# facebookresearch/foundpose

Measured on AMD Instinct MI355X. Metric: detections/sec (ViT+kNN match) on 518^2 crops vs 10k-template bank, higher is better.
Workload: dtype bf16

## Files before the change

### foundpose_amd/csrc/common.hpp

```cpp
#pragma once
#include <hip/hip_runtime.h>
#include <stdint.h>

#include <atomic>

typedef __attribute__((ext_vector_type(8))) __bf16 bf16x8;
typedef __attribute__((ext_vector_type(4))) __bf16 bf16x4;
typedef __attribute__((ext_vector_type(2))) __bf16 bf16x2;
typedef __attribute__((ext_vector_type(16))) float f32x16;
typedef __attribute__((ext_vector_type(4))) float f32x4;
typedef __attribute__((ext_vector_type(2))) float f32x2;

#define FP_DEVICE __device__ __forceinline__

enum : int {
  FP_OK = 0,
  FP_ERR_INVALID = 1,
  FP_ERR_UNSUPPORTED = 2,
  FP_ERR_HIP = 3,
};

void fp_set_error(const char* fmt, ...);

#define FP_REQUIRE(cond, ...)              \
// ... 2 lines not shown
      fp_set_error(__VA_ARGS__);           \
      return FP_ERR_INVALID;               \
    }                                      \
  } while (0)

#define FP_CHECK_LAUNCH(name)                                              \
  do {                                                                     \
    hipError_t e__ = hipGetLastError();                                    \
    if (e__ != hipSuccess) {                                               \
      fp_set_error("%s: launch failed: %s", name, hipGetErrorString(e__)); \
      return FP_ERR_HIP;                                                   \
    }                                                                      \
  } while (0)

FP_DEVICE float bf16_to_f32(__bf16 v) { return (float)v; }

FP_DEVICE float clamp448(float v) { return fminf(fmaxf(v, -448.f), 448.f); }
FP_DEVICE unsigned pack_fp8x4(float v0, float v1, float v2, float v3) {
  int w = __builtin_amdgcn_cvt_pk_fp8_f32(clamp448(v0), clamp448(v1), 0, false);
  return (unsigned)__builtin_amdgcn_cvt_pk_fp8_f32(clamp448(v2), clamp448(v3), w, true);
}
FP_DEVICE float nanmax3(float a, float b, float c) { return __builtin_elementwise_maximum(a, __builtin_elementwise_maximum(b, c)); }
FP_DEVICE unsigned pack_fp8x4(float v0, float v1, float v2, float v3, float& amax) {
  amax = nanmax3(nanmax3(amax, fabsf(v0), fabsf(v1)), fabsf(v2), fabsf(v3));
  return pack_fp8x4(v0, v1, v2, v3);
}
constexpr float FP_F16_MAX = 65504.f, FP_E4M3_MAX = 448.f;
FP_DEVICE void report_saturation(int* sat, int slot, float amax, float limit) {
  if (sat != nullptr && !(amax <= limit)) atomicAdd(sat + slot, 1);
}

FP_DEVICE unsigned pack_bf16x2(float lo, float hi) {
  f32x2 p = {lo, hi};
  return __builtin_bit_cast(unsigned, __builtin_convertvector(p, bf16x2));
}

typedef __attribute__((ext_vector_type(8))) _Float16 f16x8;
typedef __attribute__((ext_vector_type(2))) _Float16 f16x2;
FP_DEVICE unsigned pack_f16x2(float lo, float hi) {
  f32x2 p = {lo, hi};
  return __builtin_bit_cast(unsigned, __builtin_convertvector(p, f16x2));
}
template <bool H16> FP_DEVICE unsigned pack_h2(float lo, float hi) {
  if constexpr (H16) return pack_f16x2(lo, hi);
  else return pack_bf16x2(lo, hi);
}
template <bool H16> FP_DEVICE f32x2 unpack_h2(unsigned w) {
  if constexpr (H16) return __builtin_convertvector(__builtin_bit_cast(f16x2, w), f32x2);
  else return f32x2{__uint_as_float(w << 16), __uint_as_float(w & 0xffff0000u)};
}
template <bool H16> FP_DEVICE f32x16 mfma_h(bf16x8 a, bf16x8 b, f32x16 c) {
  if constexpr (H16) return __builtin_amdgcn_mfma_f32_32x32x16_f16(__builtin_bit_cast(f16x8, a), __builtin_bit_cast(f16x8, b), c, 0, 0, 0);
  else return __builtin_amdgcn_mfma_f32_32x32x16_bf16(a, b, c, 0, 0, 0);
}

FP_DEVICE void split16_pack2(float a, float b, float scale, unsigned& hi, unsigned& lo) {
  a = __builtin_amdgcn_fmed3f(a * scale, -65504.f, 65504.f);
  b = __builtin_amdgcn_fmed3f(b * scale, -65504.f, 65504.f);
  const f16x2 h = __builtin_convertvector(f32x2{a, b}, f16x2);
  const f32x2 hf = __builtin_convertvector(h, f32x2);
  const f16x2 l = __builtin_convertvector(f32x2{a - hf[0], b - hf[1]}, f16x2);
  hi = __builtin_bit_cast(unsigned, h);
  lo = __builtin_bit_cast(unsigned, l);
}
FP_DEVICE void split16_pack2_inrange(float a, float b, float scale, unsigned& hi, unsigned& lo) {
  a *= scale;
  b *= scale;
  const f16x2 h = __builtin_convertvector(f32x2{a, b}, f16x2);
  const f32x2 hf = __builtin_convertvector(h, f32x2);
  const f16x2 l = __builtin_convertvector(f32x2{a - hf[0], b - hf[1]}, f16x2);
  hi = __builtin_bit_cast(unsigned, h);
  lo = __builtin_bit_cast(unsigned, l);
}
FP_DEVICE void split16_pack2(float a, float b, float scale, unsigned& hi, unsigned& lo, float& amax) {
  amax = nanmax3(amax, fabsf(a * scale), fabsf(b * scale));
  split16_pack2(a, b, scale, hi, lo);
}
FP_DEVICE int split16_pos(int c) { return ((c >> 5) << 6) + (c & 31); }

constexpr float FP_SX_HI_SCALE = 0.0078125f, FP_SX_LO_SCALE = 16.f;
constexpr float FP_SX_MAX = 57344.f;
constexpr unsigned FP_SX_MFMA_SCALE = 0x82828282u;
FP_DEVICE int splitx_pos(int c) { return ((c >> 6) << 7) + (c & 63); }
FP_DEVICE int splitx_hi8(int c) { return ((c >> 6) << 8) + 128 + (c & 63); }
FP_DEVICE void splitx_pack2(float a, float b, float scale, unsigned& hi, unsigned& p8) {
  a = __builtin_amdgcn_fmed3f(a * scale, -65504.f, 65504.f);
  b = __builtin_amdgcn_fmed3f(b * scale, -65504.f, 65504.f);
  const f16x2 h = __builtin_convertvector(f32x2{a, b}, f16x2);
  const f32x2 hf = __builtin_convertvector(h, f32x2);
  hi = __builtin_bit_cast(unsigned, h);
  int w = __builtin_amdgcn_cvt_pk_fp8_f32(clamp448(hf[0] * FP_SX_HI_SCALE), clamp448(hf[1] * FP_SX_HI_SCALE), 0, false);
  p8 = (unsigned)__builtin_amdgcn_cvt_pk_fp8_f32(clamp448((a - hf[0]) * FP_SX_LO_SCALE), clamp448((b - hf[1]) * FP_SX_LO_SCALE), w, true);
}
FP_DEVICE void splitx_pack2(float a, float b, float scale, unsigned& hi, unsigned& p8, float& amax) {
  amax = nanmax3(amax, fabsf(a * scale), fabsf(b * scale));
  splitx_pack2(a, b, scale, hi, p8);
}
FP_DEVICE void splitx_store2(char* row, int c, unsigned hi, unsigned p8) {
  *reinterpret_cast<unsigned*>(row + splitx_pos(c) * 2) = hi;
  *reinterpret_cast<unsigned short*>(row + splitx_hi8(c)) = (unsigned short)p8;
  *reinterpret_cast<unsigned short*>(row + splitx_hi8(c) + 64) = (unsigned short)(p8 >> 16);
}
FP_DEVICE void splitx_store4(char* row, int c, unsigned hi01, unsigned p01, unsigned hi23, unsigned p23) {
  *reinterpret_cast<uint2*>(row + splitx_pos(c) * 2) = make_uint2(hi01, hi23);
  *reinterpret_cast<unsigned*>(row + splitx_hi8(c)) = __builtin_amdgcn_perm(p23, p01, 0x05040100u);
  *reinterpret_cast<unsigned*>(row + splitx_hi8(c) + 64) = __builtin_amdgcn_perm(p23, p01, 0x07060302u);
// ... 61 lines not shown
```

### foundpose_amd/csrc/gemm_bf16.hip

```cpp
#include "common.hpp"
#include "kernels.hpp"

namespace {

constexpr int BK = 64;

typedef __attribute__((address_space(3))) void lds_void;

FP_DEVICE int swz(int row) { return (row >> 1) & 7; }

FP_DEVICE unsigned stage_lane_offset(int ld, int lane, int parity) {
  const int row_l = lane >> 3;
  const int chunk = (lane & 7) ^ ((4 * parity + (row_l >> 1)) & 7);
  return (unsigned)(row_l * ld + chunk * 8) * 2u;
}
FP_DEVICE void stage_rows(__amdgpu_buffer_rsrc_t rsrc, unsigned voff, int ld, int row0, int k0, char* lds, int rblk) {
  const unsigned soff = (unsigned)((row0 + rblk * 8) * ld + k0) * 2u;
  __builtin_amdgcn_raw_ptr_buffer_load_lds(rsrc, (lds_void*)(lds + rblk * 1024), 16, voff, soff, 0, 0);
}

FP_DEVICE bf16x8 read_frag(const char* lds, int row, int chunk) {
  return *reinterpret_cast<const bf16x8*>(lds + row * 128 + ((chunk ^ swz(row)) << 4));
}

// ... 32 lines not shown
  const f32x2 phi = __builtin_elementwise_fma(xc, q, f32x2{0.5f, 0.5f});
  return x * phi;
}

FP_DEVICE f32x2 gelu_erf_pk(f32x2 x) {
  const f32x2 hx = x * f32x2{0.5f, 0.5f};
  const f32x2 hax = {__builtin_fabsf(hx[0]), __builtin_fabsf(hx[1])};
  const f32x2 z = hax * f32x2{1.41421356237309504880f, 1.41421356237309504880f};
  const f32x2 den = __builtin_elementwise_fma(z, f32x2{0.3275911f, 0.3275911f}, f32x2{1.f, 1.f});
  const f32x2 t = {__builtin_amdgcn_rcpf(den[0]), __builtin_amdgcn_rcpf(den[1])};
  f32x2 q = f32x2{-0.29844723923966754f, -0.29844723923966754f};
  q = __builtin_elementwise_fma(q, t, f32x2{1.5048025775340452f, 1.5048025775340452f});
  q = __builtin_elementwise_fma(q, t, f32x2{-2.0855161249300567f, -2.0855161249300567f});
  q = __builtin_elementwise_fma(q, t, f32x2{2.040068178110667f, 2.040068178110667f});
  q = __builtin_elementwise_fma(q, t, f32x2{-0.7490454190655901f, -0.7490454190655901f});
  q = __builtin_elementwise_fma(q, t, f32x2{0.4310967998728252f, 0.4310967998728252f});
  q = __builtin_elementwise_fma(q, t, f32x2{0.15704123123125485f, 0.15704123123125485f});
  q = q * t;
  const f32x2 a = z * (z * f32x2{-1.44269504088896340736f, -1.44269504088896340736f});
  const f32x2 e = {__builtin_amdgcn_exp2f(a[0]), __builtin_amdgcn_exp2f(a[1])};
  const f32x2 erfz = __builtin_elementwise_fma(-q, e, f32x2{1.f, 1.f});
  return __builtin_elementwise_fma(hax, erfz, hx);
}

FP_DEVICE float row32_sum(float v) {
  v += __builtin_bit_cast(float, __builtin_amdgcn_update_dpp(0, __builtin_bit_cast(int, v), 0xB1, 0xF, 0xF, true));
  v += __builtin_bit_cast(float, __builtin_amdgcn_update_dpp(0, __builtin_bit_cast(int, v), 0x4E, 0xF, 0xF, true));
  v += __builtin_bit_cast(float, __builtin_amdgcn_update_dpp(0, __builtin_bit_cast(int, v), 0x124, 0xF, 0xF, true));
  v += __builtin_bit_cast(float, __builtin_amdgcn_update_dpp(0, __builtin_bit_cast(int, v), 0x128, 0xF, 0xF, true));
  v += __builtin_bit_cast(float, __builtin_amdgcn_update_dpp(0, __builtin_bit_cast(int, v), 0x142, 0xA, 0xF, true));
  return v;
}

FP_DEVICE float row16_sum(float v) {
  v += __builtin_bit_cast(float, __builtin_amdgcn_update_dpp(0, __builtin_bit_cast(int, v), 0xB1, 0xF, 0xF, true));
  v += __builtin_bit_cast(float, __builtin_amdgcn_update_dpp(0, __builtin_bit_cast(int, v), 0x4E, 0xF, 0xF, true));
  v += __builtin_bit_cast(float, __builtin_amdgcn_update_dpp(0, __builtin_bit_cast(int, v), 0x124, 0xF, 0xF, true));
  v += __builtin_bit_cast(float, __builtin_amdgcn_update_dpp(0, __builtin_bit_cast(int, v), 0x128, 0xF, 0xF, true));
  return v;
}

typedef __attribute__((ext_vector_type(8))) int i32x8;
typedef __attribute__((ext_vector_type(4))) int i32x4;

template <int EPI, int BM, int BN, int WM, int WN, bool F8 = false, bool F8OUT = false, bool SP = false, bool SPOUT = false, bool SX = false, bool H16 = false, int NSTAGE = 2>
__global__ __launch_bounds__(WM * WN * 64, 2) void gemm_bf16_kernel(GemmBf16Args a) {
  static_assert(!SX || SP, "f16f8 rows are a form of the split operands");
  static_assert(NSTAGE == 2 || (NSTAGE == 4 && !F8 && !SP && WM * WN != 8), "the deep pipeline exists for the small bf16 / fp16 tiles");
  static_assert(!H16 || (!F8 && !SP), "plain fp16 operands exclude the fp8 and the split forms");
  static_assert(!F8OUT || (F8 && (EPI == GEMM_EPI_GELU_BF16 || EPI == GEMM_EPI_SWIGLU_BF16)), "fp8 output: GELU / SwiGLU epilogues of the fp8 kernels");
  static_assert(!(SP && F8) && (!SPOUT || SP), "split-fp16 and fp8 operands exclude each other; a split output needs split operands");
  static_assert(SPOUT == (SP && (EPI == GEMM_EPI_BIAS_BF16 || EPI == GEMM_EPI_GELU_BF16 || EPI == GEMM_EPI_SWIGLU_BF16)), "f16x3: the half-precision epilogues write split rows");
  constexpr int NW = WM * WN, NT = NW * 64, TM = BM / WM / 32, TN = BN / WN / 32;
  constexpr bool HILO = EPI == GEMM_EPI_RESID_HILO;
  constexpr bool RESID = EPI == GEMM_EPI_LS_RESID_F32 || EPI == GEMM_EPI_RESID_F32 || HILO;
  constexpr int A_BYTES = BM * BK * 2, B_BYTES = BN * BK * 2, STAGE = A_BYTES + B_BYTES;
  constexpr bool ASYM = NW == 8;
  constexpr int NISSUE = ASYM ? NW / 2 : NW;
  constexpr int A_INSTR = BM / 8 / NISSUE, B_INSTR = BN / 8 / NISSUE;
  constexpr int PIECES = A_INSTR + B_INSTR;
  static_assert(PIECES % 2 == 0, "staging split");
  extern __shared__ __attribute__((aligned(16))) char smem[];
  const int tid = threadIdx.x, lane = tid & 63, wave = __builtin_amdgcn_readfirstlane(tid >> 6);
  const int wm = wave / WN, wn = wave % WN, l31 = lane & 31, kh = lane >> 5;

  const unsigned nwg = gridDim.x;
  const unsigned lid = xcd_remap(blockIdx.x, nwg);
  const unsigned tiles_n = a.N / BN;
  int m0, n0;
  if (a.rast_r) {
    const unsigned per = a.rast_r * a.rast_gn, st = lid / per, r = lid - st * per;
    const unsigned SM = (a.m_tiles + a.rast_r - 1) / a.rast_r;
    const unsigned sn = st / SM, sm = st - sn * SM;
    const unsigned tm = sm * a.rast_r + r % a.rast_r, tn = sn * a.rast_gn + r / a.rast_r;
    if (tm >= (unsigned)a.m_tiles) return;
    m0 = tm * BM;
    n0 = tn * BN;
  } else {
    m0 = (lid / tiles_n) * BM;
    n0 = (lid % tiles_n) * BN;
  }
  const int kb = 0, ke = a.K / BK;

#ifdef FP_GEMM_TIMELINE
  unsigned long long ts0 = 0, ts1 = 0, ts2 = 0;
  if (a.dbg) ts0 = __builtin_readcyclecounter();
#endif
  {
    f32x16 acc[TM][TN];
#pragma unroll
    for (int i = 0; i < TM; ++i)
#pragma unroll
      for (int j = 0; j < TN; ++j)
#pragma unroll
        for (int r = 0; r < 16; ++r) acc[i][j][r] = 0.f;

    static_assert(A_INSTR % 2 == 0 && B_INSTR % 2 == 0, "row-group parity of a piece must be a compile-time property");
    auto tile_rsrc = [](const __bf16* base, int row0, int rows, int ld) {
      const unsigned long long bytes = (unsigned long long)(rows - row0) * ld * 2ull;
      return __builtin_amdgcn_make_buffer_rsrc((void*)(base + (size_t)row0 * ld), 0, bytes > 0xffffffffull ? 0xffffffffu : (unsigned)bytes, 0x00020000);
    };
    const __amdgpu_buffer_rsrc_t rsrc_a = tile_rsrc(a.A, m0, a.M, a.lda), rsrc_w = tile_rsrc(a.W, n0, a.N, a.ldw);
    const unsigned voff_a[2] = {stage_lane_offset(a.lda, lane, 0), stage_lane_offset(a.lda, lane, 1)};
    const unsigned voff_w[2] = {stage_lane_offset(a.ldw, lane, 0), stage_lane_offset(a.ldw, lane, 1)};
    const bool issuer = !ASYM || wm == 0;
    const int iw = ASYM ? wave % NISSUE : wave;
    auto stage_piece = [&](int q, int t, char* buf) {
      if (!issuer) return;
      if (q < A_INSTR) stage_rows(rsrc_a, voff_a[q & 1], a.lda, 0, t * BK, buf, iw * A_INSTR + q);
      else stage_rows(rsrc_w, voff_w[(q - A_INSTR) & 1], a.ldw, 0, t * BK, buf + A_BYTES, iw * B_INSTR + (q - A_INSTR));
    };
#pragma unroll
    for (int q = 0; q < PIECES; ++q) stage_piece(q, kb, smem);
    if constexpr (NSTAGE > 2) {
#pragma unroll
      for (int d = 1; d < NSTAGE - 1; ++d)
        if (kb + d < ke) {
#pragma unroll
          for (int q = 0; q < PIECES; ++q) stage_piece(q, kb + d, smem + d * STAGE);
        }
    }

    float ln_rs[TM], ln_mrs[TM];
#pragma unroll
    for (int i = 0; i < TM; ++i) { ln_rs[i] = 1.f; ln_mrs[i] = 0.f; }
    if constexpr (!F8 && (EPI == GEMM_EPI_BIAS_BF16 || EPI == GEMM_EPI_GELU_BF16 || EPI == GEMM_EPI_SWIGLU_BF16)) {
      if (a.ln_stats) {
#pragma unroll
        for (int i = 0; i < TM; ++i) {
          const float2 st = a.ln_stats[m0 + wm * (BM / WM) + i * 32 + l31];
          ln_rs[i] = st.x;
          ln_mrs[i] = st.y;
          if constexpr (H16) {
            ln_rs[i] *= a.acc_scale;
            ln_mrs[i] *= a.acc_scale;
          }
        }
      }
    }

    {
      for (int t = kb; t < ke; ++t) {
        const int cur = NSTAGE == 2 ? ((t - kb) & 1) : ((t - kb) % NSTAGE);
        if constexpr (NSTAGE == 2) {
          asm volatile("s_waitcnt vmcnt(0)" ::: "memory");
        } else {
          static_assert((NSTAGE - 2) * PIECES == 12, "s_waitcnt immediate below");
          if (t + NSTAGE - 2 < ke) asm volatile("s_waitcnt vmcnt(12)" ::: "memory");
          else asm volatile("s_waitcnt vmcnt(0)" ::: "memory");
        }
        __syncthreads();
#ifdef FP_GEMM_TIMELINE
        if (a.dbg && t == 0) ts1 = __builtin_readcyclecounter();
#endif
        char* nxt = smem + (NSTAGE == 2 ? (cur ^ 1) : ((t - kb + NSTAGE - 1) % NSTAGE)) * STAGE;
        const bool more = t + (NSTAGE - 1) < ke;
        const char* As = smem + cur * STAGE;
        const char* Ws = As + A_BYTES;
        if constexpr (F8) {
#pragma unroll
          for (int s = 0; s < 2; ++s) {
            if (more) {
#pragma unroll
              for (int q = 0; q < PIECES / 2; ++q) stage_piece(s * (PIECES / 2) + q, t + 1, nxt);
            }
            const int chunk = s * 4 + kh * 2;
            __builtin_amdgcn_iglp_opt(1);
            i32x8 af[TM], wf[TN];
            auto frag8 = [&](const char* base, int row) {
              const i32x4 lo = __builtin_bit_cast(i32x4, read_frag(base, row, chunk));
              const i32x4 hi = __builtin_bit_cast(i32x4, read_frag(base, row, chunk + 1));
              return __builtin_shufflevector(lo, hi, 0, 1, 2, 3, 4, 5, 6, 7);
            };
#pragma unroll
            for (int i = 0; i < TM; ++i) af[i] = frag8(As, wm * (BM / WM) + i * 32 + l31);
#pragma unroll
            for (int j = 0; j < TN; ++j) wf[j] = frag8(Ws, wn * (BN / WN) + j * 32 + l31);
#pragma unroll
            for (int i = 0; i < TM; ++i)
#pragma unroll
              for (int j = 0; j < TN; ++j)
                acc[i][j] = __builtin_amdgcn_mfma_scale_f32_32x32x64_f8f6f4(wf[j], af[i], acc[i][j], 0, 0, 0, 0x7f7f7f7f, 0, 0x7f7f7f7f);
          }
// ... 35 lines not shown
                const i32x4 lo = __builtin_bit_cast(i32x4, read_frag(base, row, chunk));
                const i32x4 hi = __builtin_bit_cast(i32x4, read_frag(base, row, chunk + 1));
                return __builtin_shufflevector(lo, hi, 0, 1, 2, 3, 4, 5, 6, 7);
              };
#pragma unroll
              for (int i = 0; i < TM; ++i) af[i] = frag8(As1, wm * (BM / WM) + i * 32 + l31, ca);
#pragma unroll
              for (int j = 0; j < TN; ++j) wf[j] = frag8(Ws1, wn * (BN / WN) + j * 32 + l31, cw);
#pragma unroll
              for (int i = 0; i < TM; ++i)
#pragma unroll
                for (int j = 0; j < TN; ++j)
                  acc[i][j] = __builtin_amdgcn_mfma_scale_f32_32x32x64_f8f6f4(wf[j], af[i], acc[i][j], 0, 0, 0, (int)FP_SX_MFMA_SCALE, 0, 0x7f7f7f7f);
            }
            ++t;
          }
        } else if constexpr (SP) {
#pragma unroll
          for (int s2 = 0; s2 < 2; ++s2) {
            if (more) {
#pragma unroll
              for (int q = 0; q < PIECES / 2; ++q) stage_piece(s2 * (PIECES / 2) + q, t + 1, nxt);
            }
            const int ch = s2 * 2 + kh;
            __builtin_amdgcn_iglp_opt(1);
            f16x8 ah[TM], al[TM], wh[TN], wl[TN];
#pragma unroll
            for (int i = 0; i < TM; ++i) {
              const int row = wm * (BM / WM) + i * 32 + l31;
              ah[i] = __builtin_bit_cast(f16x8, read_frag(As, row, ch));
              al[i] = __builtin_bit_cast(f16x8, read_frag(As, row, ch + 4));
            }
#pragma unroll
            for (int j = 0; j < TN; ++j) {
              const int row = wn * (BN / WN) + j * 32 + l31;
              wh[j] = __builtin_bit_cast(f16x8, read_frag(Ws, row, ch));
              wl[j] = __builtin_bit_cast(f16x8, read_frag(Ws, row, ch + 4));
            }
#pragma unroll
            for (int i = 0; i < TM; ++i)
#pragma unroll
              for (int j = 0; j < TN; ++j) acc[i][j] = __builtin_amdgcn_mfma_f32_32x32x16_f16(wl[j], ah[i], acc[i][j], 0, 0, 0);
#pragma unroll
            for (int i = 0; i < TM; ++i)
#pragma unroll
              for (int j = 0; j < TN; ++j) acc[i][j] = __builtin_amdgcn_mfma_f32_32x32x16_f16(wh[j], al[i], acc[i][j], 0, 0, 0);
#pragma unroll
            for (int i = 0; i < TM; ++i)
#pragma unroll
              for (int j = 0; j < TN; ++j) acc[i][j] = __builtin_amdgcn_mfma_f32_32x32x16_f16(wh[j], ah[i], acc[i][j], 0, 0, 0);
          }
        } else {
#pragma unroll
        for (int ks = 0; ks < 4; ++ks) {
          if (more) {
#pragma unroll
            for (int q = (ks * PIECES) / 4; q < ((ks + 1) * PIECES) / 4; ++q) stage_piece(q, t + (NSTAGE - 1), nxt);
          }
          const int chunk = ks * 2 + kh;
          if constexpr (TM * TN >= 4) __builtin_amdgcn_iglp_opt(1);
          bf16x8 af[TM], wf[TN];
#pragma unroll
          for (int i = 0; i < TM; ++i) af[i] = read_frag(As, wm * (BM / WM) + i * 32 + l31, chunk);
#pragma unroll
          for (int j = 0; j < TN; ++j) wf[j] = read_frag(Ws, wn * (BN / WN) + j * 32 + l31, chunk);
#pragma unroll
          for (int i = 0; i < TM; ++i)
#pragma unroll
            for (int j = 0; j < TN; ++j)
              acc[i][j] = mfma_h<H16>(wf[j], af[i], acc[i][j]);
        }
      }
        }
      __syncthreads();
    }
#ifdef FP_GEMM_TIMELINE
    if (a.dbg) ts2 = __builtin_readcyclecounter();
#endif

    constexpr bool USE_SLAB = EPI == GEMM_EPI_BIAS_BF16 || EPI == GEMM_EPI_GELU_BF16 ||
                              EPI == GEMM_EPI_SWIGLU_BF16 || RESID;
    static_assert(!F8 || USE_SLAB, "the fp8 kernels exist for the slab epilogues only");
    if constexpr (USE_SLAB) {
    constexpr bool OUT_F32 = RESID || EPI == GEMM_EPI_TOKENS_F32 || EPI == GEMM_EPI_BIAS_F32;
    constexpr int ESZ = OUT_F32 ? 4 : (F8OUT ? 1 : (SPOUT ? 4 : 2));
    constexpr int OUT_COLS = EPI == GEMM_EPI_SWIGLU_BF16 ? BN / 2 : BN;
    constexpr int SLAB_ROWS = WM * 32, SLAB_STRIDE = OUT_COLS * ESZ + 16;
    constexpr int CHUNKS_PER_ROW = OUT_COLS * ESZ / 16, SLAB_CHUNKS = SLAB_ROWS * CHUNKS_PER_ROW, NT = NW * 64;
    static_assert(SLAB_ROWS * SLAB_STRIDE <= 2 * STAGE, "slab must fit the main-loop LDS");
    constexpr bool TWO_SLABS = 2 * SLAB_ROWS * SLAB_STRIDE <= 2 * STAGE;
    constexpr int SLAB_BYTES = SLAB_ROWS * SLAB_STRIDE;
    constexpr bool LN_FOLD_OK = !F8 && (EPI == GEMM_EPI_BIAS_BF16 || EPI == GEMM_EPI_GELU_BF16 || EPI == GEMM_EPI_SWIGLU_BF16);
    const bool fold = LN_FOLD_OK && a.ln_stats != nullptr;
    float4 bias[TN][4], gam[TN][4];
  #pragma unroll
    for (int tn = 0; tn < TN; ++tn)
  #pragma unroll
      for (int g = 0; g < 4; ++g) {
        const int n = n0 + wn * (BN / WN) + tn * 32 + 8 * g + 4 * kh;
        bias[tn][g] = *reinterpret_cast<const float4*>(a.bias + n);
        if constexpr (EPI == GEMM_EPI_LS_RESID_F32 || F8) gam[tn][g] = *reinterpret_cast<const float4*>(a.gamma + n);
        if constexpr (LN_FOLD_OK) {
          if (fold) gam[tn][g] = *reinterpret_cast<const float4*>(a.colsum + n);
        }
      }
    __syncthreads();
    float sat_amax = 0.f;
  #pragma unroll
    for (int tm = 0; tm < TM; ++tm) {
      const int m = m0 + wm * (BM / WM) + tm * 32 + l31;
      float band_amax = 0.f;
      constexpr int PASSES = (SLAB_CHUNKS + NT - 1) / NT;
      static_assert(SLAB_CHUNKS % NT == 0, "slab chunks must divide evenly over the block");
      float4 ext[PASSES];
      int orow_i[PASSES];
      constexpr int CPR8 = HILO ? OUT_COLS / 8 : 1, PASS8 = HILO ? SLAB_ROWS * CPR8 / NT : 1;
      uint4 exh[PASS8], exl[PASS8];
      if constexpr (HILO) {
        static_assert(!HILO || (SLAB_ROWS * CPR8) % NT == 0, "slab chunks must divide evenly over the block");
  #pragma unroll
        for (int it = 0; it < PASS8; ++it) {
          const int id = tid + it * NT;
          const int r = id / CPR8, c = id - r * CPR8;
          const int gm_row = m0 + (r >> 5) * (BM / WM) + tm * 32 + (r & 31);
          const bool okr = gm_row < a.M_valid;
          if (okr) {
            exh[it] = *reinterpret_cast<const uint4*>(a.xb + (size_t)gm_row * a.ld_xb + n0 + c * 8);
            exl[it] = *reinterpret_cast<const uint4*>(a.xl + (size_t)gm_row * a.ld_xb + n0 + c * 8);
          }
          orow_i[it] = okr ? gm_row : -1;
        }
      }
  #pragma unroll
      for (int it = 0; it < (HILO ? 0 : PASSES); ++it) {
        const int id = tid + it * NT;
        const int r = id / CHUNKS_PER_ROW, c = id - r * CHUNKS_PER_ROW;
        const int gm_row = m0 + (r >> 5) * (BM / WM) + tm * 32 + (r & 31);
        const bool okr = gm_row < a.M_valid;
        int orow = gm_row;
        if constexpr (EPI == GEMM_EPI_TOKENS_F32) {
          const int b = gm_row / a.tok_np, pidx = gm_row - b * a.tok_np;
          orow = b * a.tok_n + a.tok_skip + pidx;
          if (okr) ext[it] = *reinterpret_cast<const float4*>(a.pos + (size_t)pidx * a.ldo + n0 + c * 4);
        }
        if constexpr (RESID) {
          if (okr) ext[it] = *reinterpret_cast<const float4*>(reinterpret_cast<const float*>(a.out) + (size_t)orow * a.ldo + n0 + c * 4);
        }
        orow_i[it] = okr ? orow : -1;
      }
      const float rs = ln_rs[tm], mrs = ln_mrs[tm];
      char* slab = smem + (TWO_SLABS ? (tm & 1) * SLAB_BYTES : 0);
      char* srow = slab + (wm * 32 + l31) * SLAB_STRIDE;
  #pragma unroll
      for (int tn = 0; tn < TN; ++tn)
  #pragma unroll
        for (int g = 0; g < 4; ++g) {
          const int col = wn * (BN / WN) + tn * 32 + 8 * g + 4 * kh;
          const float4 bs = bias[tn][g];
          float v0 = acc[tm][tn][4 * g + 0] + bs.x, v1 = acc[tm][tn][4 * g + 1] + bs.y;
          float v2 = acc[tm][tn][4 * g + 2] + bs.z, v3 = acc[tm][tn][4 * g + 3] + bs.w;
          if constexpr (SP || H16) {
            const float as = a.acc_scale;
            v0 = fmaf(acc[tm][tn][4 * g + 0], as, bs.x); v1 = fmaf(acc[tm][tn][4 * g + 1], as, bs.y);
            v2 = fmaf(acc[tm][tn][4 * g + 2], as, bs.z); v3 = fmaf(acc[tm][tn][4 * g + 3], as, bs.w);
          }
          if constexpr (LN_FOLD_OK) {
            if (fold) {
              const float4 cs = gam[tn][g];
              const f32x2 rs2 = {rs, rs}, nm2 = {-mrs, -mrs};
              const f32x2 t01 = __builtin_elementwise_fma(nm2, f32x2{cs.x, cs.y}, f32x2{bs.x, bs.y});
              const f32x2 t23 = __builtin_elementwise_fma(nm2, f32x2{cs.z, cs.w}, f32x2{bs.z, bs.w});
              const f32x2 r01 = __builtin_elementwise_fma(rs2, f32x2{acc[tm][tn][4 * g + 0], acc[tm][tn][4 * g + 1]}, t01);
              const f32x2 r23 = __builtin_elementwise_fma(rs2, f32x2{acc[tm][tn][4 * g + 2], acc[tm][tn][4 * g + 3]}, t23);
              v0 = r01[0]; v1 = r01[1]; v2 = r23[0]; v3 = r23[1];
            }
          }
          if constexpr (F8 && EPI != GEMM_EPI_LS_RESID_F32) {
            const float4 gm = gam[tn][g];
            v0 *= gm.x; v1 *= gm.y; v2 *= gm.z; v3 *= gm.w;
          }
          if constexpr (EPI == GEMM_EPI_GELU_BF16) {
            if constexpr (H16) {
              const f32x2 g01 = gelu_pk9(f32x2{v0, v1}), g23 = gelu_pk9(f32x2{v2, v3});
              v0 = g01[0]; v1 = g01[1]; v2 = g23[0]; v3 = g23[1];
            } else if constexpr (SP) {
              const f32x2 g01 = gelu_erf_pk(f32x2{v0, v1}), g23 = gelu_erf_pk(f32x2{v2, v3});
              v0 = g01[0]; v1 = g01[1]; v2 = g23[0]; v3 = g23[1];
            } else {
              const f32x2 g01 = gelu_pk(f32x2{v0, v1}), g23 = gelu_pk(f32x2{v2, v3});
              v0 = g01[0]; v1 = g01[1]; v2 = g23[0]; v3 = g23[1];
            }
          }
          if constexpr (EPI == GEMM_EPI_LS_RESID_F32) {
            const float4 gm = gam[tn][g];
            v0 *= gm.x; v1 *= gm.y; v2 *= gm.z; v3 *= gm.w;
          }
          if constexpr (EPI == GEMM_EPI_SWIGLU_BF16) {
            float h0, h1;
            if constexpr (SP) {
              h0 = v0 / (1.f + expf(-v0)) * v1;
              h1 = v2 / (1.f + expf(-v2)) * v3;
            } else {
              h0 = v0 / (1.f + __builtin_amdgcn_exp2f(-v0 * 1.44269504088896340736f)) * v1;
              h1 = v2 / (1.f + __builtin_amdgcn_exp2f(-v2 * 1.44269504088896340736f)) * v3;
            }
            if constexpr (SPOUT && SX) {
              unsigned hi, p8;
              splitx_pack2(h0, h1, a.out_scale, hi, p8, band_amax);
              splitx_store2(srow, col >> 1, hi, p8);
            } else if constexpr (SPOUT) {
              unsigned hi, lo;
              split16_pack2(h0, h1, a.out_scale, hi, lo, band_amax);
              char* sp = srow + split16_pos(col >> 1) * 2;
              *reinterpret_cast<unsigned*>(sp) = hi;
              *reinterpret_cast<unsigned*>(sp + 64) = lo;
            } else if constexpr (F8OUT) *reinterpret_cast<unsigned short*>(srow + (col >> 1)) = (unsigned short)pack_fp8x4(h0 * a.out_scale, h1 * a.out_scale, 0.f, 0.f, band_amax);
            else *reinterpret_cast<unsigned*>(srow + (col >> 1) * 2) = pack_h2<H16>(h0, h1);
          } else if constexpr (SPOUT && SX && EPI != GEMM_EPI_BIAS_BF16) {
            unsigned h01, p01, h23, p23;
            splitx_pack2(v0, v1, a.out_scale, h01, p01, band_amax);
            splitx_pack2(v2, v3, a.out_scale, h23, p23, band_amax);
            splitx_store4(srow, col, h01, p01, h23, p23);
          } else if constexpr (SPOUT) {
            unsigned h01, l01, h23, l23;
            split16_pack2(v0, v1, a.out_scale, h01, l01, band_amax);
            split16_pack2(v2, v3, a.out_scale, h23, l23, band_amax);
            char* sp = srow + split16_pos(col) * 2;
            *reinterpret_cast<uint2*>(sp) = make_uint2(h01, h23);
            *reinterpret_cast<uint2*>(sp + 64) = make_uint2(l01, l23);
          } else if constexpr (OUT_F32) *reinterpret_cast<float4*>(srow + col * 4) = make_float4(v0, v1, v2, v3);
          else if constexpr (F8OUT) *reinterpret_cast<unsigned*>(srow + col) = pack_fp8x4(v0 * a.out_scale, v1 * a.out_scale, v2 * a.out_scale, v3 * a.out_scale, band_amax);
          else *reinterpret_cast<uint2*>(srow + col * 2) = make_uint2(pack_h2<H16>(v0, v1), pack_h2<H16>(v2, v3));
        }
      if constexpr (SPOUT || F8OUT) {
        if (m < a.M_valid) sat_amax = nanmax3(sat_amax, band_amax, 0.f);
      }
      __syncthreads();
      if constexpr (HILO) {
  #pragma unroll
        for (int it = 0; it < PASS8; ++it) {
          const int id = tid + it * NT;
          const int r = id / CPR8, c = id - r * CPR8;
          if (orow_i[it] < 0) continue;
          const size_t orow_it = (size_t)orow_i[it];
          const char* sp = slab + r * SLAB_STRIDE + c * 32;
          const float4 s0 = *reinterpret_cast<const float4*>(sp), s1v = *reinterpret_cast<const float4*>(sp + 16);
          const unsigned hw[4] = {exh[it].x, exh[it].y, exh[it].z, exh[it].w}, lw[4] = {exl[it].x, exl[it].y, exl[it].z, exl[it].w};
          float v[8] = {s0.x, s0.y, s0.z, s0.w, s1v.x, s1v.y, s1v.z, s1v.w};
          unsigned ho[4], lo[4];
          float s1 = 0.f, s2 = 0.f;
  #pragma unroll
          for (int q = 0; q < 4; ++q) {
            const f32x2 xh = unpack_h2<H16>(hw[q]), xlo = unpack_h2<H16>(lw[q]);
            v[2 * q] += xh[0] + xlo[0];
            v[2 * q + 1] += xh[1] + xlo[1];
            ho[q] = pack_h2<H16>(v[2 * q], v[2 * q + 1]);
            const f32x2 nh = unpack_h2<H16>(ho[q]);
            lo[q] = pack_h2<H16>(v[2 * q] - nh[0], v[2 * q + 1] - nh[1]);
            s1 += v[2 * q] + v[2 * q + 1];
            s2 += fmaf(v[2 * q], v[2 * q], v[2 * q + 1] * v[2 * q + 1]);
          }
          *reinterpret_cast<uint4*>(a.xb + orow_it * a.ld_xb + n0 + c * 8) = make_uint4(ho[0], ho[1], ho[2], ho[3]);
          *reinterpret_cast<uint4*>(a.xl + orow_it * a.ld_xb + n0 + c * 8) = make_uint4(lo[0], lo[1], lo[2], lo[3]);
          s1 = row16_sum(s1);
          s2 = row16_sum(s2);
          if ((c & 15) == 15) a.stats_out[(size_t)(n0 / 128 + (c >> 4)) * a.M + orow_it] = make_float2(s1, s2);
        }
      }
  #pragma unroll
      for (int it = 0; it < (HILO ? 0 : PASSES); ++it) {
        const int id = tid + it * NT;
        const int r = id / CHUNKS_PER_ROW, c = id - r * CHUNKS_PER_ROW;
        if (orow_i[it] < 0) continue;
        const size_t orow_it = (size_t)orow_i[it];
        const char* sp = slab + r * SLAB_STRIDE + c * 16;
        if constexpr (F8OUT) {
          const int ncol = (EPI == GEMM_EPI_SWIGLU_BF16 ? n0 / 2 : n0) + c * 16;
          *reinterpret_cast<uint4*>(reinterpret_cast<unsigned char*>(a.out) + orow_it * a.ldo + ncol) = *reinterpret_cast<const uint4*>(sp);
        } else if constexpr (!OUT_F32) {
          const int ncol = (EPI == GEMM_EPI_SWIGLU_BF16 ? n0 / 2 : n0) * (SPOUT ? 2 : 1) + c * 8;
          *reinterpret_cast<uint4*>(reinterpret_cast<__bf16*>(a.out) + orow_it * a.ldo + ncol) = *reinterpret_cast<const uint4*>(sp);
        } else {
          float4 v = *reinterpret_cast<const float4*>(sp);
          if constexpr (RESID || EPI == GEMM_EPI_TOKENS_F32) {
            v.x += ext[it].x; v.y += ext[it].y; v.z += ext[it].z; v.w += ext[it].w;
          }
          *reinterpret_cast<float4*>(reinterpret_cast<float*>(a.out) + orow_it * a.ldo + n0 + c * 4) = v;
          if constexpr (EPI == GEMM_EPI_RESID_F32 && !F8) {
            if (a.xb) {
              *reinterpret_cast<uint2*>(a.xb + orow_it * a.ld_xb + n0 + c * 4) = make_uint2(pack_h2<H16>(v.x, v.y), pack_h2<H16>(v.z, v.w));
              float s1 = (v.x + v.y) + (v.z + v.w), s2 = fmaf(v.x, v.x, v.y * v.y) + fmaf(v.z, v.z, v.w * v.w);
              s1 = row32_sum(s1);
              s2 = row32_sum(s2);
              if ((c & 31) == 31) a.stats_out[(size_t)(n0 / 128 + (c >> 5)) * a.M + orow_it] = make_float2(s1, s2);
            }
          }
        }
      }
      if (!TWO_SLABS && tm + 1 < TM) __syncthreads();
    }
    if constexpr (SPOUT) report_saturation(a.sat, 0, sat_amax, (SX && EPI != GEMM_EPI_BIAS_BF16) ? FP_SX_MAX : FP_F16_MAX);
    if constexpr (F8OUT) report_saturation(a.sat, 1, sat_amax, FP_E4M3_MAX);
    } else {
    float4 bias[TN][4], gam[TN][4];
  #pragma unroll
    for (int tn = 0; tn < TN; ++tn)
  #pragma unroll
      for (int g = 0; g < 4; ++g) {
        const int n = n0 + wn * (BN / WN) + tn * 32 + 8 * g + 4 * kh;
        bias[tn][g] = *reinterpret_cast<const float4*>(a.bias + n);
        if constexpr (EPI == GEMM_EPI_LS_RESID_F32) gam[tn][g] = *reinterpret_cast<const float4*>(a.gamma + n);
      }
  #pragma unroll
    for (int tm = 0; tm < TM; ++tm) {
      const int m = m0 + wm * (BM / WM) + tm * 32 + l31;
      if (m >= a.M_valid) continue;
      size_t out_row = m;
      int pidx = 0;
      if constexpr (EPI == GEMM_EPI_TOKENS_F32) {
        const int b = m / a.tok_np;
        pidx = m - b * a.tok_np;
        out_row = (size_t)b * a.tok_n + a.tok_skip + pidx;
      }
      float4 extra[TN][4];
      if constexpr (EPI == GEMM_EPI_LS_RESID_F32 || EPI == GEMM_EPI_TOKENS_F32) {
  #pragma unroll
        for (int tn = 0; tn < TN; ++tn)
  #pragma unroll
          for (int g = 0; g < 4; ++g) {
            const int n = n0 + wn * (BN / WN) + tn * 32 + 8 * g + 4 * kh;
            if constexpr (EPI == GEMM_EPI_LS_RESID_F32)
              extra[tn][g] = *reinterpret_cast<const float4*>(reinterpret_cast<const float*>(a.out) + out_row * a.ldo + n);
            else
              extra[tn][g] = *reinterpret_cast<const float4*>(a.pos + (size_t)pidx * a.ldo + n);
          }
      }
  #pragma unroll
      for (int tn = 0; tn < TN; ++tn)
  #pragma unroll
        for (int g = 0; g < 4; ++g) {
          const int n = n0 + wn * (BN / WN) + tn * 32 + 8 * g + 4 * kh;
          const float4 bs = bias[tn][g];
          float v0 = acc[tm][tn][4 * g + 0] + bs.x, v1 = acc[tm][tn][4 * g + 1] + bs.y;
          float v2 = acc[tm][tn][4 * g + 2] + bs.z, v3 = acc[tm][tn][4 * g + 3] + bs.w;
          if constexpr (SP || H16) {
            const float as = a.acc_scale;
            v0 = fmaf(acc[tm][tn][4 * g + 0], as, bs.x); v1 = fmaf(acc[tm][tn][4 * g + 1], as, bs.y);
            v2 = fmaf(acc[tm][tn][4 * g + 2], as, bs.z); v3 = fmaf(acc[tm][tn][4 * g + 3], as, bs.w);
          }
          if constexpr (EPI == GEMM_EPI_BIAS_BF16 || EPI == GEMM_EPI_GELU_BF16) {
            if constexpr (EPI == GEMM_EPI_GELU_BF16) {
              const f32x2 g01 = gelu_pk(f32x2{v0, v1}), g23 = gelu_pk(f32x2{v2, v3});
              v0 = g01[0]; v1 = g01[1]; v2 = g23[0]; v3 = g23[1];
            }
            uint2 pk = make_uint2(pack_h2<H16>(v0, v1), pack_h2<H16>(v2, v3));
            *reinterpret_cast<uint2*>(reinterpret_cast<__bf16*>(a.out) + out_row * a.ldo + n) = pk;
          } else if constexpr (EPI == GEMM_EPI_LS_RESID_F32) {
            const float4 gm = gam[tn][g];
            float4 x = extra[tn][g];
            x.x += gm.x * v0; x.y += gm.y * v1; x.z += gm.z * v2; x.w += gm.w * v3;
            *reinterpret_cast<float4*>(reinterpret_cast<float*>(a.out) + out_row * a.ldo + n) = x;
          } else if constexpr (EPI == GEMM_EPI_TOKENS_F32) {
            const float4 pe = extra[tn][g];
            *reinterpret_cast<float4*>(reinterpret_cast<float*>(a.out) + out_row * a.ldo + n) =
                make_float4(v0 + pe.x, v1 + pe.y, v2 + pe.z, v3 + pe.w);
          } else if constexpr (EPI == GEMM_EPI_BIAS_F32) {
            *reinterpret_cast<float4*>(reinterpret_cast<float*>(a.out) + out_row * a.ldo + n) = make_float4(v0, v1, v2, v3);
          }
        }
    }
    }
#ifdef FP_GEMM_TIMELINE
    if (a.dbg) {
      asm volatile("s_waitcnt vmcnt(0)" ::: "memory");
      const unsigned long long ts3 = __builtin_readcyclecounter();
      if (tid == 0) {
        unsigned long long* d = a.dbg + (size_t)blockIdx.x * 4;
        d[0] = ts0; d[1] = ts1; d[2] = ts2; d[3] = ts3;
      }
    }
#endif
  }
}

struct GemmRaster { int r, gn; };
static GemmRaster pick_raster(int bm, int n_tiles, unsigned grid) {
  const int wide8 = n_tiles % 8 == 0;
  const int rr = wide8 ? 4 : 8, gn = wide8 ? 8 : 4;
  if (bm >= 256 && n_tiles % gn == 0 && n_tiles > 4 && grid >= 512) return {rr, gn};
  return {0, 0};
}

template <int EPI, int BM, int BN, int WM, int WN, bool F8 = false, bool F8OUT = false, bool SP = false, bool SPOUT = false, bool SX = false, bool H16 = false, int NSTAGE = 2>
int launch_cfg(const GemmBf16Args& a_in, hipStream_t st) {
  GemmBf16Args a = a_in;
  if constexpr (H16) {
    if (!(a.acc_scale > 0.f)) a.acc_scale = 1.f;
  }
  a.m_tiles = a.M / BM;
  if (a.M_valid > 0 && (a.M_valid + BM - 1) / BM < a.m_tiles) a.m_tiles = (a.M_valid + BM - 1) / BM;
  unsigned grid = a.m_tiles * (a.N / BN);
  a.rast_r = a.rast_gn = 0;
  const GemmRaster ra = pick_raster(BM, a.N / BN, grid);
  if (ra.r) {
    a.rast_r = ra.r; a.rast_gn = ra.gn;
    grid = ((a.m_tiles + ra.r - 1) / ra.r) * ((a.N / BN) / ra.gn) * 32;
  }
  const size_t lds = (size_t)(BM + BN) * BK * 2 * NSTAGE;
  static FpDeviceOnce attr;
  fp_allow_dynamic_lds(attr, &gemm_bf16_kernel<EPI, BM, BN, WM, WN, F8, F8OUT, SP, SPOUT, SX, H16, NSTAGE>, (int)lds);
  hipLaunchKernelGGL((gemm_bf16_kernel<EPI, BM, BN, WM, WN, F8, F8OUT, SP, SPOUT, SX, H16, NSTAGE>), dim3(grid), dim3(WM * WN * 64), lds, st, a);
  FP_CHECK_LAUNCH("gemm_bf16_kernel");
  return FP_OK;
}

static int xcd_rounds(int bm, int m_valid, int n_tiles) {
// ... 129 lines not shown
```

Baseline: 1143.

## Use 16x16x32 MFMA tiles for plain bf16/f16 GEMM paths

```diff
diff --git a/foundpose_amd/csrc/common.hpp b/foundpose_amd/csrc/common.hpp
--- a/foundpose_amd/csrc/common.hpp
+++ b/foundpose_amd/csrc/common.hpp
@@ -78,6 +78,10 @@
 template <bool H16> FP_DEVICE f32x16 mfma_h(bf16x8 a, bf16x8 b, f32x16 c) {
   if constexpr (H16) return __builtin_amdgcn_mfma_f32_32x32x16_f16(__builtin_bit_cast(f16x8, a), __builtin_bit_cast(f16x8, b), c, 0, 0, 0);
   else return __builtin_amdgcn_mfma_f32_32x32x16_bf16(a, b, c, 0, 0, 0);
+}
+template <bool H16> FP_DEVICE f32x4 mfma16_h(bf16x8 a, bf16x8 b, f32x4 c) {
+  if constexpr (H16) return __builtin_amdgcn_mfma_f32_16x16x32_f16(__builtin_bit_cast(f16x8, a), __builtin_bit_cast(f16x8, b), c, 0, 0, 0);
+  else return __builtin_amdgcn_mfma_f32_16x16x32_bf16(a, b, c, 0, 0, 0);
 }
 
 FP_DEVICE void split16_pack2(float a, float b, float scale, unsigned& hi, unsigned& lo) {
diff --git a/foundpose_amd/csrc/gemm_bf16.hip b/foundpose_amd/csrc/gemm_bf16.hip
--- a/foundpose_amd/csrc/gemm_bf16.hip
+++ b/foundpose_amd/csrc/gemm_bf16.hip
@@ -108,6 +108,11 @@
   static_assert(!(SP && F8) && (!SPOUT || SP), "split-fp16 and fp8 operands exclude each other; a split output needs split operands");
   static_assert(SPOUT == (SP && (EPI == GEMM_EPI_BIAS_BF16 || EPI == GEMM_EPI_GELU_BF16 || EPI == GEMM_EPI_SWIGLU_BF16)), "f16x3: the half-precision epilogues write split rows");
   constexpr int NW = WM * WN, NT = NW * 64, TM = BM / WM / 32, TN = BN / WN / 32;
+  constexpr bool M16 = !F8 && !SP;
+  constexpr int MT = M16 ? 16 : 32;
+  constexpr int TMI = BM / WM / MT, TNI = BN / WN / MT;
+  using AccT = std::conditional_t<M16, f32x4, f32x16>;
+  constexpr int ACC_N = M16 ? 4 : 16;
   constexpr bool HILO = EPI == GEMM_EPI_RESID_HILO;
   constexpr bool RESID = EPI == GEMM_EPI_LS_RESID_F32 || EPI == GEMM_EPI_RESID_F32 || HILO;
   constexpr int A_BYTES = BM * BK * 2, B_BYTES = BN * BK * 2, STAGE = A_BYTES + B_BYTES;
@@ -119,6 +124,7 @@
   extern __shared__ __attribute__((aligned(16))) char smem[];
   const int tid = threadIdx.x, lane = tid & 63, wave = __builtin_amdgcn_readfirstlane(tid >> 6);
   const int wm = wave / WN, wn = wave % WN, l31 = lane & 31, kh = lane >> 5;
+  const int lrow = M16 ? lane & 15 : l31, lcol = M16 ? 4 * (lane >> 4) : 4 * kh;
 
   const unsigned nwg = gridDim.x;
   const unsigned lid = xcd_remap(blockIdx.x, nwg);
@@ -143,13 +149,13 @@
   if (a.dbg) ts0 = __builtin_readcyclecounter();
 #endif
   {
-    f32x16 acc[TM][TN];
-#pragma unroll
-    for (int i = 0; i < TM; ++i)
-#pragma unroll
-      for (int j = 0; j < TN; ++j)
-#pragma unroll
-        for (int r = 0; r < 16; ++r) acc[i][j][r] = 0.f;
+    AccT acc[TMI][TNI];
+#pragma unroll
+    for (int i = 0; i < TMI; ++i)
+#pragma unroll
+      for (int j = 0; j < TNI; ++j)
+#pragma unroll
+        for (int r = 0; r < ACC_N; ++r) acc[i][j][r] = 0.f;
 
     static_assert(A_INSTR % 2 == 0 && B_INSTR % 2 == 0, "row-group parity of a piece must be a compile-time property");
     auto tile_rsrc = [](const __bf16* base, int row0, int rows, int ld) {
@@ -177,14 +183,17 @@
         }
     }
 
-    float ln_rs[TM], ln_mrs[TM];
-#pragma unroll
-    for (int i = 0; i < TM; ++i) { ln_rs[i] = 1.f; ln_mrs[i] = 0.f; }
+    constexpr int LN_N = M16 ? (TMI + 3) / 4 : TMI;
+    float ln_rs[LN_N], ln_mrs[LN_N];
+#pragma unroll
+    for (int i = 0; i < LN_N; ++i) { ln_rs[i] = 1.f; ln_mrs[i] = 0.f; }
     if constexpr (!F8 && (EPI == GEMM_EPI_BIAS_BF16 || EPI == GEMM_EPI_GELU_BF16 || EPI == GEMM_EPI_SWIGLU_BF16)) {
       if (a.ln_stats) {
 #pragma unroll
-        for (int i = 0; i < TM; ++i) {
-          const float2 st = a.ln_stats[m0 + wm * (BM / WM) + i * 32 + l31];
+        for (int i = 0; i < LN_N; ++i) {
+          const int rb = M16 ? 4 * i + (lane >> 4) : i;
+          if (M16 && rb >= TMI) continue;
+          const float2 st = a.ln_stats[m0 + wm * (BM / WM) + rb * MT + lrow];
           ln_rs[i] = st.x;
           ln_mrs[i] = st.y;
           if constexpr (H16) {
@@ -326,23 +335,22 @@
           }
         } else {
 #pragma unroll
-        for (int ks = 0; ks < 4; ++ks) {
+        for (int ks = 0; ks < 2; ++ks) {
           if (more) {
 #pragma unroll
-            for (int q = (ks * PIECES) / 4; q < ((ks + 1) * PIECES) / 4; ++q) stage_piece(q, t + (NSTAGE - 1), nxt);
-          }
-          const int chunk = ks * 2 + kh;
-          if constexpr (TM * TN >= 4) __builtin_amdgcn_iglp_opt(1);
-          bf16x8 af[TM], wf[TN];
-#pragma unroll
-          for (int i = 0; i < TM; ++i) af[i] = read_frag(As, wm * (BM / WM) + i * 32 + l31, chunk);
-#pragma unroll
-          for (int j = 0; j < TN; ++j) wf[j] = read_frag(Ws, wn * (BN / WN) + j * 32 + l31, chunk);
-#pragma unroll
-          for (int i = 0; i < TM; ++i)
-#pragma unroll
-            for (int j = 0; j < TN; ++j)
-              acc[i][j] = mfma_h<H16>(wf[j], af[i], acc[i][j]);
+            for (int q = (ks * PIECES) / 2; q < ((ks + 1) * PIECES) / 2; ++q) stage_piece(q, t + (NSTAGE - 1), nxt);
+          }
+          const int chunk = ks * 4 + (lane >> 4);
+          if constexpr (TMI * TNI >= 16) __builtin_amdgcn_iglp_opt(1);
+          bf16x8 wf[TNI];
+#pragma unroll
+          for (int j = 0; j < TNI; ++j) wf[j] = read_frag(Ws, wn * (BN / WN) + j * 16 + lrow, chunk);
+#pragma unroll
+          for (int i = 0; i < TMI; ++i) {
+            const bf16x8 af = read_frag(As, wm * (BM / WM) + i * 16 + lrow, chunk);
+#pragma unroll
+            for (int j = 0; j < TNI; ++j) acc[i][j] = mfma16_h<H16>(wf[j], af, acc[i][j]);
+          }
         }
       }
         }
@@ -352,6 +360,12 @@
     if (a.dbg) ts2 = __builtin_readcyclecounter();
 #endif
 
+    constexpr int CGW = M16 ? 16 : 8, NCG = BN / WN / CGW;
+    constexpr int RPB = 32 / MT;
+    auto acc4 = [&](int rb, int cg) -> f32x4 {
+      if constexpr (M16) return acc[rb][cg];
+      else return f32x4{acc[rb][cg >> 2][4 * (cg & 3) + 0], acc[rb][cg >> 2][4 * (cg & 3) + 1], acc[rb][cg >> 2][4 * (cg & 3) + 2], acc[rb][cg >> 2][4 * (cg & 3) + 3]};
+    };
     constexpr bool USE_SLAB = EPI == GEMM_EPI_BIAS_BF16 || EPI == GEMM_EPI_GELU_BF16 ||
                               EPI == GEMM_EPI_SWIGLU_BF16 || RESID;
     static_assert(!F8 || USE_SLAB, "the fp8 kernels exist for the slab epilogues only");
@@ -366,18 +380,16 @@
     constexpr int SLAB_BYTES = SLAB_ROWS * SLAB_STRIDE;
     constexpr bool LN_FOLD_OK = !F8 && (EPI == GEMM_EPI_BIAS_BF16 || EPI == GEMM_EPI_GELU_BF16 || EPI == GEMM_EPI_SWIGLU_BF16);
     const bool fold = LN_FOLD_OK && a.ln_stats != nullptr;
-    float4 bias[TN][4], gam[TN][4];
-  #pragma unroll
-    for (int tn = 0; tn < TN; ++tn)
-  #pragma unroll
-      for (int g = 0; g < 4; ++g) {
-        const int n = n0 + wn * (BN / WN) + tn * 32 + 8 * g + 4 * kh;
-        bias[tn][g] = *reinterpret_cast<const float4*>(a.bias + n);
-        if constexpr (EPI == GEMM_EPI_LS_RESID_F32 || F8) gam[tn][g] = *reinterpret_cast<const float4*>(a.gamma + n);
-        if constexpr (LN_FOLD_OK) {
-          if (fold) gam[tn][g] = *reinterpret_cast<const float4*>(a.colsum + n);
-        }
-      }
+    float4 bias[NCG], gam[NCG];
+  #pragma unroll
+    for (int cg = 0; cg < NCG; ++cg) {
+      const int n = n0 + wn * (BN / WN) + cg * CGW + lcol;
+      bias[cg] = *reinterpret_cast<const float4*>(a.bias + n);
+      if constexpr (EPI == GEMM_EPI_LS_RESID_F32 || F8) gam[cg] = *reinterpret_cast<const float4*>(a.gamma + n);
+      if constexpr (LN_FOLD_OK) {
+        if (fold) gam[cg] = *reinterpret_cast<const float4*>(a.colsum + n);
+      }
+    }
     __syncthreads();
     float sat_amax = 0.f;
   #pragma unroll
@@ -422,35 +434,49 @@
         }
         orow_i[it] = okr ? orow : -1;
       }
-      const float rs = ln_rs[tm], mrs = ln_mrs[tm];
       char* slab = smem + (TWO_SLABS ? (tm & 1) * SLAB_BYTES : 0);
-      char* srow = slab + (wm * 32 + l31) * SLAB_STRIDE;
-  #pragma unroll
-      for (int tn = 0; tn < TN; ++tn)
-  #pragma unroll
-        for (int g = 0; g < 4; ++g) {
-          const int col = wn * (BN / WN) + tn * 32 + 8 * g + 4 * kh;
-          const float4 bs = bias[tn][g];
-          float v0 = acc[tm][tn][4 * g + 0] + bs.x, v1 = acc[tm][tn][4 * g + 1] + bs.y;
-          float v2 = acc[tm][tn][4 * g + 2] + bs.z, v3 = acc[tm][tn][4 * g + 3] + bs.w;
+  #pragma unroll
+      for (int s = 0; s < RPB; ++s) {
+      const int rb = tm * RPB + s;
+      float rs = 1.f, mrs = 0.f;
+      if constexpr (LN_FOLD_OK) {
+        if (fold) {
+          if constexpr (M16) {
+            const int src = (lane & 15) + 16 * (rb & 3);
+            rs = __shfl(ln_rs[rb >> 2], src, 64);
+            mrs = __shfl(ln_mrs[rb >> 2], src, 64);
+          } else {
+            rs = ln_rs[rb];
+            mrs = ln_mrs[rb];
+          }
+        }
+      }
+      char* srow = slab + (wm * 32 + s * MT + lrow) * SLAB_STRIDE;
+  #pragma unroll
+      for (int cg = 0; cg < NCG; ++cg) {
+          const int col = wn * (BN / WN) + cg * CGW + lcol;
+          const float4 bs = bias[cg];
+          const f32x4 c4 = acc4(rb, cg);
+          float v0 = c4[0] + bs.x, v1 = c4[1] + bs.y;
+          float v2 = c4[2] + bs.z, v3 = c4[3] + bs.w;
           if constexpr (SP || H16) {
             const float as = a.acc_scale;
-            v0 = fmaf(acc[tm][tn][4 * g + 0], as, bs.x); v1 = fmaf(acc[tm][tn][4 * g + 1], as, bs.y);
-            v2 = fmaf(acc[tm][tn][4 * g + 2], as, bs.z); v3 = fmaf(acc[tm][tn][4 * g + 3], as, bs.w);
+            v0 = fmaf(c4[0], as, bs.x); v1 = fmaf(c4[1], as, bs.y);
+            v2 = fmaf(c4[2], as, bs.z); v3 = fmaf(c4[3], as, bs.w);
           }
           if constexpr (LN_FOLD_OK) {
             if (fold) {
-              const float4 cs = gam[tn][g];
+              const float4 cs = gam[cg];
               const f32x2 rs2 = {rs, rs}, nm2 = {-mrs, -mrs};
               const f32x2 t01 = __builtin_elementwise_fma(nm2, f32x2{cs.x, cs.y}, f32x2{bs.x, bs.y});
               const f32x2 t23 = __builtin_elementwise_fma(nm2, f32x2{cs.z, cs.w}, f32x2{bs.z, bs.w});
-              const f32x2 r01 = __builtin_elementwise_fma(rs2, f32x2{acc[tm][tn][4 * g + 0], acc[tm][tn][4 * g + 1]}, t01);
-              const f32x2 r23 = __builtin_elementwise_fma(rs2, f32x2{acc[tm][tn][4 * g + 2], acc[tm][tn][4 * g + 3]}, t23);
+              const f32x2 r01 = __builtin_elementwise_fma(rs2, f32x2{c4[0], c4[1]}, t01);
+              const f32x2 r23 = __builtin_elementwise_fma(rs2, f32x2{c4[2], c4[3]}, t23);
               v0 = r01[0]; v1 = r01[1]; v2 = r23[0]; v3 = r23[1];
             }
           }
           if constexpr (F8 && EPI != GEMM_EPI_LS_RESID_F32) {
-            const float4 gm = gam[tn][g];
+            const float4 gm = gam[cg];
             v0 *= gm.x; v1 *= gm.y; v2 *= gm.z; v3 *= gm.w;
           }
           if constexpr (EPI == GEMM_EPI_GELU_BF16) {
@@ -466,7 +492,7 @@
             }
           }
           if constexpr (EPI == GEMM_EPI_LS_RESID_F32) {
-            const float4 gm = gam[tn][g];
+            const float4 gm = gam[cg];
             v0 *= gm.x; v1 *= gm.y; v2 *= gm.z; v3 *= gm.w;
           }
           if constexpr (EPI == GEMM_EPI_SWIGLU_BF16) {
@@ -506,6 +532,7 @@
           else if constexpr (F8OUT) *reinterpret_cast<unsigned*>(srow + col) = pack_fp8x4(v0 * a.out_scale, v1 * a.out_scale, v2 * a.out_scale, v3 * a.out_scale, band_amax);
           else *reinterpret_cast<uint2*>(srow + col * 2) = make_uint2(pack_h2<H16>(v0, v1), pack_h2<H16>(v2, v3));
         }
+      }
       if constexpr (SPOUT || F8OUT) {
         if (m < a.M_valid) sat_amax = nanmax3(sat_amax, band_amax, 0.f);
       }
@@ -576,18 +603,16 @@
     if constexpr (SPOUT) report_saturation(a.sat, 0, sat_amax, (SX && EPI != GEMM_EPI_BIAS_BF16) ? FP_SX_MAX : FP_F16_MAX);
     if constexpr (F8OUT) report_saturation(a.sat, 1, sat_amax, FP_E4M3_MAX);
     } else {
-    float4 bias[TN][4], gam[TN][4];
-  #pragma unroll
-    for (int tn = 0; tn < TN; ++tn)
-  #pragma unroll
-      for (int g = 0; g < 4; ++g) {
-        const int n = n0 + wn * (BN / WN) + tn * 32 + 8 * g + 4 * kh;
-        bias[tn][g] = *reinterpret_cast<const float4*>(a.bias + n);
-        if constexpr (EPI == GEMM_EPI_LS_RESID_F32) gam[tn][g] = *reinterpret_cast<const float4*>(a.gamma + n);
-      }
-  #pragma unroll
-    for (int tm = 0; tm < TM; ++tm) {
-      const int m = m0 + wm * (BM / WM) + tm * 32 + l31;
+    float4 bias[NCG], gam[NCG];
+  #pragma unroll
+    for (int cg = 0; cg < NCG; ++cg) {
+      const int n = n0 + wn * (BN / WN) + cg * CGW + lcol;
+      bias[cg] = *reinterpret_cast<const float4*>(a.bias + n);
+      if constexpr (EPI == GEMM_EPI_LS_RESID_F32) gam[cg] = *reinterpret_cast<const float4*>(a.gamma + n);
+    }
+  #pragma unroll
+    for (int rb = 0; rb < TMI; ++rb) {
+      const int m = m0 + wm * (BM / WM) + rb * MT + lrow;
       if (m >= a.M_valid) continue;
       size_t out_row = m;
       int pidx = 0;
@@ -596,31 +621,28 @@
         pidx = m - b * a.tok_np;
         out_row = (size_t)b * a.tok_n + a.tok_skip + pidx;
       }
-      float4 extra[TN][4];
+      float4 extra[NCG];
       if constexpr (EPI == GEMM_EPI_LS_RESID_F32 || EPI == GEMM_EPI_TOKENS_F32) {
   #pragma unroll
-        for (int tn = 0; tn < TN; ++tn)
-  #pragma unroll
-          for (int g = 0; g < 4; ++g) {
-            const int n = n0 + wn * (BN / WN) + tn * 32 + 8 * g + 4 * kh;
-            if constexpr (EPI == GEMM_EPI_LS_RESID_F32)
-              extra[tn][g] = *reinterpret_cast<const float4*>(reinterpret_cast<const float*>(a.out) + out_row * a.ldo + n);
-            else
-              extra[tn][g] = *reinterpret_cast<const float4*>(a.pos + (size_t)pidx * a.ldo + n);
-          }
-      }
-  #pragma unroll
-      for (int tn = 0; tn < TN; ++tn)
-  #pragma unroll
-        for (int g = 0; g < 4; ++g) {
-          const int n = n0 + wn * (BN / WN) + tn * 32 + 8 * g + 4 * kh;
-          const float4 bs = bias[tn][g];
-          float v0 = acc[tm][tn][4 * g + 0] + bs.x, v1 = acc[tm][tn][4 * g + 1] + bs.y;
-          float v2 = acc[tm][tn][4 * g + 2] + bs.z, v3 = acc[tm][tn][4 * g + 3] + bs.w;
+        for (int cg = 0; cg < NCG; ++cg) {
+          const int n = n0 + wn * (BN / WN) + cg * CGW + lcol;
+          if constexpr (EPI == GEMM_EPI_LS_RESID_F32)
+            extra[cg] = *reinterpret_cast<const float4*>(reinterpret_cast<const float*>(a.out) + out_row * a.ldo + n);
+          else
+            extra[cg] = *reinterpret_cast<const float4*>(a.pos + (size_t)pidx * a.ldo + n);
+        }
+      }
+  #pragma unroll
+      for (int cg = 0; cg < NCG; ++cg) {
+          const int n = n0 + wn * (BN / WN) + cg * CGW + lcol;
+          const float4 bs = bias[cg];
+          const f32x4 c4 = acc4(rb, cg);
+          float v0 = c4[0] + bs.x, v1 = c4[1] + bs.y;
+          float v2 = c4[2] + bs.z, v3 = c4[3] + bs.w;
           if constexpr (SP || H16) {
             const float as = a.acc_scale;
-            v0 = fmaf(acc[tm][tn][4 * g + 0], as, bs.x); v1 = fmaf(acc[tm][tn][4 * g + 1], as, bs.y);
-            v2 = fmaf(acc[tm][tn][4 * g + 2], as, bs.z); v3 = fmaf(acc[tm][tn][4 * g + 3], as, bs.w);
+            v0 = fmaf(c4[0], as, bs.x); v1 = fmaf(c4[1], as, bs.y);
+            v2 = fmaf(c4[2], as, bs.z); v3 = fmaf(c4[3], as, bs.w);
           }
           if constexpr (EPI == GEMM_EPI_BIAS_BF16 || EPI == GEMM_EPI_GELU_BF16) {
             if constexpr (EPI == GEMM_EPI_GELU_BF16) {
@@ -630,12 +652,12 @@
             uint2 pk = make_uint2(pack_h2<H16>(v0, v1), pack_h2<H16>(v2, v3));
             *reinterpret_cast<uint2*>(reinterpret_cast<__bf16*>(a.out) + out_row * a.ldo + n) = pk;
           } else if constexpr (EPI == GEMM_EPI_LS_RESID_F32) {
-            const float4 gm = gam[tn][g];
-            float4 x = extra[tn][g];
+            const float4 gm = gam[cg];
+            float4 x = extra[cg];
             x.x += gm.x * v0; x.y += gm.y * v1; x.z += gm.z * v2; x.w += gm.w * v3;
             *reinterpret_cast<float4*>(reinterpret_cast<float*>(a.out) + out_row * a.ldo + n) = x;
           } else if constexpr (EPI == GEMM_EPI_TOKENS_F32) {
-            const float4 pe = extra[tn][g];
+            const float4 pe = extra[cg];
             *reinterpret_cast<float4*>(reinterpret_cast<float*>(a.out) + out_row * a.ldo + n) =
                 make_float4(v0 + pe.x, v1 + pe.y, v2 + pe.z, v3 + pe.w);
           } else if constexpr (EPI == GEMM_EPI_BIAS_F32) {
```

Result: no change. 1163, median of 6 (+1.7%).
